# hohMiyazawa/hoh-ANS

Hardware: AMD Instinct MI355X
Metric: MB/s encode+decode (bit-exact) on 8-bit RGB, 1/2/4/8 MI355X; % HBM roofline (higher is better)
Workload: dtype u8; 1 GPU; 8192x8192 synthetic RGB (gradient + triangular noise k=4, seeds 1..32: one image each), 256x256 tiles, choh -s0 encode + dhoh decode, side index, 4 slot(s) x 8 image(s) per step (batched calls hoh_encode_images_async / hoh_decode_images_async) = 32 images in flight per GPU, 4 hardware queues; W=8192, H=8192, tiles=1024, per_gpu=8192x8192, batch=8, parallelism=1 GPU

## Files before the change

hoh-ans_amd/csrc/hoh_api.cpp:

```cpp
#include "hoh_internal.h"
#include "hoh_dec.h"
#include "hoh_index_blob.h"
#include "../../include/hoh_ans.h"

#include <math.h>
#include <string.h>
#include <stdlib.h>
#include <vector>
#include <algorithm>
#include <stdio.h>
#include <string>
#include <atomic>

void launch_synth(uint8_t* rgb, int W, int H, int y0, uint64_t seed, int noise, hipStream_t s);
void launch_natural(uint8_t* rgb, int W, int rows, int y0, uint64_t seed, hipStream_t s);
void launch_put_bytes(uint8_t* dst, const uint8_t* b, int n, hipStream_t s, int copies = 1, uint64_t stride = 0);
void launch_status_enc(const uint32_t* gerr, const uint64_t* total, uint64_t cap, uint64_t* out, hipStream_t s);
void launch_status_enc_batch(const uint32_t* gerr, const uint64_t* img_total, const uint32_t* img_err,
                             uint64_t stride, uint64_t* out, int n, hipStream_t s);

std::atomic<uint64_t> g_device_allocs{0};

namespace {

// ... 80 lines not shown
      c->sms[k] += v;
      c->scount[k] += 1;
    }
  }
  c->nmark = 0;
  c->knames.clear();
}

static void prof_mark(hoh_ctx* c, hipStream_t s, const char* name, bool reset) {
  if (!c->profiling) return;
  if (reset) prof_fold(c);
  if (c->nmark == c->kev.size()) {
    hipEvent_t e;
    if (hipEventCreate(&e) != hipSuccess) return;
    c->kev.push_back(e);
  }
  (void)hipEventRecord(c->kev[c->nmark++], s);
  c->knames.push_back(name);
}

struct Prof {
  hoh_ctx* c;
  hipStream_t s;
  Prof(hoh_ctx* c_, hipStream_t s_, bool async = false) : c(c_), s(s_) { prof_mark(c, s, "start", !async); }
  void mark(const char* name) { prof_mark(c, s, name, false); }
};

extern "C" {

const char* hoh_version(void) { return "hoh-ans_amd 0.2 (gfx950)"; }

uint64_t hoh_device_alloc_count(void) { return g_device_allocs.load(std::memory_order_relaxed); }

const char* hoh_strerror(int code) {
  switch (code) {
    case HOH_OK: return "ok";
    case HOH_E_ARG: return "invalid argument";
    case HOH_E_CAP: return "output capacity too small";
    case HOH_E_HIP: return "HIP runtime error";
    case HOH_E_RANGE: return "symbol / range / prob_bits outside the supported set";
    case HOH_E_UNREPRODUCIBLE: return "the reference emits uninitialised bytes for this input";
    case HOH_E_UNSUPPORTED: return "not implemented on this path";
    case HOH_E_CORRUPT: return "malformed or undecodable bitstream";
    case HOH_E_NODEV: return "no HIP device";
  }
  return "unknown error";
}

int hoh_ctx_create(hoh_ctx** out, int device) {
  if (!out) return HOH_E_ARG;
  *out = nullptr;
  int n = 0;
  if (hipGetDeviceCount(&n) != hipSuccess || n <= device || device < 0) return HOH_E_NODEV;
  if (hipSetDevice(device) != hipSuccess) return HOH_E_NODEV;
  {
    static std::atomic<int> warned{0};
    const char* q = getenv("GPU_MAX_HW_QUEUES");
    if (q && atoi(q) > 20 && !getenv("HOH_QUIET") && !warned.exchange(1))
      fprintf(stderr, "hoh: GPU_MAX_HW_QUEUES=%s: more than 20 hardware queues per process cost 15-30%% "
                      "throughput on MI355X; share queues between streams instead\n", q);
  }
  hoh_ctx* c = new hoh_ctx();
  c->device = device;
  if (hipDeviceGetAttribute(&c->cus, hipDeviceAttributeMultiprocessorCount, device) != hipSuccess || c->cus <= 0)
    c->cus = 256;
  if (hipStreamCreateWithFlags(&c->own, hipStreamNonBlocking) != hipSuccess) { delete c; return HOH_E_HIP; }
  if (hipHostMalloc((void**)&c->pinned, 4096) != hipSuccess) { delete c; return HOH_E_HIP; }
  *out = c;
  return HOH_OK;
}

static int lz_posting() { return HOH_KNOB(LZ_POSTING, 1); }

static void freebuf(Buf& b) { if (b.p) (void)hipFree(b.p); b.p = nullptr; b.n = 0; }

void hoh_ctx_destroy(hoh_ctx* c) {
  if (!c) return;
  (void)hipSetDevice(c->device);
  Buf* all[] = {&c->dbg, &c->idx8, &c->fpb, &c->lzs, &c->pinfo, &c->lg, &c->sym, &c->hist, &c->candbits, &c->matches, &c->lzspec, &c->pal, &c->streams, &c->tiles, &c->hdr,
                &c->tab_fast, &c->tab_gen, &c->slabs, &c->ckpt, &c->misc, &c->tsizes};
  for (Buf* b : all) freebuf(*b);
  for (Buf& b : c->scr.chunks) freebuf(b);
  dec_free(c->dec);
  for (auto e : c->kev) (void)hipEventDestroy(e);
  if (c->pinned) (void)hipHostFree(c->pinned);
  if (c->own) (void)hipStreamDestroy(c->own);
  if (c->side.s) (void)hipStreamDestroy(c->side.s);
  if (c->side.fork) (void)hipEventDestroy(c->side.fork);
  if (c->side.join) (void)hipEventDestroy(c->side.join);
  delete c;
}

void hoh_set_profiling(hoh_ctx* c, int on) { if (c) c->profiling = on; }

void* hoh_ctx_stream(hoh_ctx* c) { return c ? (void*)c->own : nullptr; }

int hoh_ctx_set_option(hoh_ctx* c, int option, int64_t value) {
  if (!c) return HOH_E_ARG;
  switch (option) {
    case HOH_OPT_NOIX_DECODER:
      if (value < HOH_NOIX_ADAPTIVE || value > HOH_NOIX_WAVE) return HOH_E_ARG;
      c->noix = (int)value;
      return HOH_OK;
    case HOH_OPT_DECODABLE:
      if (value != 0 && value != 1) return HOH_E_ARG;
      c->decodable = (int)value;
      return HOH_OK;
    case HOH_OPT_SMALL_IMAGES:
      if (value != 0 && value != 1) return HOH_E_ARG;
      c->small = (int)value;
      return HOH_OK;
    case HOH_OPT_CHAIN_TABLES:
      if (value < HOH_CHAIN_TABLES_AUTO || value > HOH_CHAIN_TABLES_GLOBAL) return HOH_E_ARG;
      c->chain_tables = (int)value;
      return HOH_OK;
  }
  return HOH_E_ARG;
}

int hoh_get_kernel_ms(hoh_ctx* c, const char** names, float* ms, int max) {
  if (!c || c->nmark < 2) return 0;
  int k = 0;
  (void)hipEventSynchronize(c->kev[c->nmark - 1]);
  for (size_t i = 1; i < c->nmark && k < max; i++, k++) {
    float v = 0;
    (void)hipEventElapsedTime(&v, c->kev[i - 1], c->kev[i]);
    if (names) names[k] = c->knames[i].c_str();
    if (ms) ms[k] = v;
  }
  return k;
}

int hoh_get_kernel_stats(hoh_ctx* c, const char** names, double* total_ms, uint64_t* count, int max) {
  if (!c) return 0;
  prof_fold(c);
  int k = 0;
  for (; k < (int)c->snames.size() && k < max; k++) {
    if (names) names[k] = c->snames[k].c_str();
    if (total_ms) total_ms[k] = c->sms[k];
    if (count) count[k] = c->scount[k];
  }
  return k;
}

#ifdef HOH_DEBUG_READ
extern "C" int hoh_debug_read(hoh_ctx* c, int which, void* dst, size_t bytes) {
  if (!c || !dst) return HOH_E_ARG;
  if (which == 2) {
    if (!c->dec.bufs[15] || bytes > c->dec.sizes[15]) return HOH_E_ARG;
    return hipMemcpy(dst, (const uint8_t*)c->dec.bufs[15] + c->dec.sizes[15] - bytes, bytes, hipMemcpyDeviceToHost) == hipSuccess
               ? HOH_OK : HOH_E_HIP;
  }
  const Buf& b = which == 0 ? c->matches : which == 3 ? c->lzs : which == 4 ? c->fpb : which == 5 ? c->dbg
               : which == 6 ? c->streams : c->lzspec;
  if (bytes > b.n || !b.p) return HOH_E_ARG;
  return hipMemcpy(dst, b.p, bytes, hipMemcpyDeviceToHost) == hipSuccess ? HOH_OK : HOH_E_HIP;
}
#endif

void hoh_reset_kernel_stats(hoh_ctx* c) {
  if (!c) return;
  prof_fold(c);
  c->snames.clear();
  c->sms.clear();
  c->scount.clear();
}

int hoh_tiling(int W, int H, int* xt, int* yt, int* tw, int* th) {
  if ((W >= 512 || H >= 512) && W >= 256 && H >= 256) {
    *xt = W / 256; *yt = H / 256;
    *tw = (W + *xt - 1) / *xt; *th = (H + *yt - 1) / *yt;
    return 1;
  }
  *xt = *yt = 1; *tw = W; *th = H;
  return 0;
}

size_t hoh_encode_bound(int W, int H) {
  int xt, yt, tw, th;
  hoh_tiling(W, H, &xt, &yt, &tw, &th);
  return 64 + (size_t)xt * yt * 3 + 5 * (size_t)W * H + (size_t)xt * yt * 4096;
}

static size_t header_fixed(int W, int H, uint8_t* o) {
  size_t p = 0;
  o[p++] = 153; o[p++] = 72; o[p++] = 79; o[p++] = 72;
  o[p++] = 2;
  o[p++] = 8;
  p = hoh_write_varint(o, (uint32_t)p, (uint64_t)W - 1);
  p = hoh_write_varint(o, (uint32_t)p, (uint64_t)H - 1);
  return p;
}

size_t hoh_file_prefix(int W, int H, const uint32_t* ts, int nt, uint8_t* out, size_t cap) {
  int xt, yt, tw, th;
  if (!hoh_tiling(W, H, &xt, &yt, &tw, &th) || nt != xt * yt) return 0;
  std::vector<uint8_t> b(32 + 3 * (size_t)nt);
  size_t p = header_fixed(W, H, b.data());
  b[p++] = (uint8_t)(xt - 1);
  b[p++] = (uint8_t)(yt - 1);
  for (int i = 0; i + 1 < nt; i++) p = hoh_write_varint(b.data(), (uint32_t)p, ts[i]);
  if (p > cap) return 0;
  memcpy(out, b.data(), p);
  return p;
}

int hoh_peek_header(const uint8_t* h, size_t size, int* W, int* H, int* xt, int* yt) {
  if (!h || size < 8 || h[0] != 153 || h[1] != 72 || h[2] != 79 || h[3] != 72) return HOH_E_CORRUPT;
  if (h[4] != 2 || h[5] != 8) return HOH_E_UNSUPPORTED;
  size_t p = 6;
  auto rv = [&](uint64_t& v) -> bool {
    if (p >= size) return false;
    uint64_t b0 = h[p++];
    if (!(b0 & 0x80)) { v = b0; return true; }
    if (p >= size) return false;
    uint64_t b1 = h[p++];
    if (!(b1 & 0x80)) { v = ((b0 & 0x7f) << 7) + b1; return true; }
    if (p >= size) return false;
    uint64_t b2 = h[p++];
    v = ((b0 & 0x7f) << 14) + ((b1 & 0x7f) << 7) + b2;
    return true;
  };
  uint64_t w, hh;
  if (!rv(w) || !rv(hh)) return HOH_E_CORRUPT;
  *W = (int)w + 1; *H = (int)hh + 1;
  int tw, th, x, y;
  hoh_tiling(*W, *H, &x, &y, &tw, &th);
  if (xt) *xt = x;
  if (yt) *yt = y;
  return HOH_OK;
}


static void prof_cb(void* p, const char* name) { ((Prof*)p)->mark(name); }

static int ensure_log2_tables(hoh_ctx* c, int W, int H, EncodeJob& j) {
  const int rw = W - (j.xt - 1) * j.tw, bh = H - (j.yt - 1) * j.th;
  uint32_t ns[4] = {(uint32_t)(j.tw * j.th), (uint32_t)(rw * j.th), (uint32_t)(j.tw * bh), (uint32_t)(rw * bh)};
  uint32_t un[4] = {0, 0, 0, 0};
  int nu = 0;
  for (int i = 0; i < 4; i++) {
    bool dup = false;
    for (int k = 0; k < nu; k++) dup |= un[k] == ns[i];
    if (!dup && ns[i]) un[nu++] = ns[i];
  }
  if (!(c->lg_key[0] == un[0] && c->lg_key[1] == un[1] && c->lg_key[2] == un[2] && c->lg_key[3] == un[3])) {
    std::vector<double> tab;
    for (int k = 0; k < nu; k++) {
      c->lg_off[k] = tab.size();
      for (uint32_t f = 0; f <= un[k] + 1; f++) tab.push_back(f ? -log2((double)f / (double)un[k]) : 0.0);
    }
    int e = ensure(c->lg, tab.size() * sizeof(double));
    if (e) return e;
    if (hipMemcpy(c->lg.p, tab.data(), tab.size() * sizeof(double), hipMemcpyHostToDevice) != hipSuccess) return HOH_E_HIP;
    for (int k = 0; k < 4; k++) c->lg_key[k] = un[k];
  }
  j.lg = (const double*)c->lg.p;
  for (int k = 0; k < 4; k++) { j.lg_n[k] = c->lg_key[k]; j.lg_off[k] = c->lg_off[k]; }
  return HOH_OK;
}

static int encode_tiles_impl(hoh_ctx* c, const uint8_t* d_rgb, int W, int H, int t0, int ntiles,
                             uint8_t* d_out, size_t cap, uint64_t prefix, int write_table,
                             uint32_t* d_tile_sizes, uint64_t* total_out, hoh_index* idx,
                             hipStream_t s, int speed = 0, uint64_t* d_status = nullptr, int nimg = 1,
                             uint64_t out_stride = 0, int small_n = 0) {
  const bool async = d_status != nullptr;
  int xt, yt, tw, th;
  hoh_tiling(W, H, &xt, &yt, &tw, &th);
  if (small_n > 0) { xt = 1; yt = small_n; tw = W; th = H / small_n; }
  if (tw > HOH_MAX_TILE_W || (size_t)tw * th > (1u << 24)) return HOH_E_UNSUPPORTED;
  if (speed && ((size_t)((tw + 39) / 40) * ((th + 39) / 40) > HOH_MAPCAP || tw > 1024)) return HOH_E_UNSUPPORTED;
  if (t0 < 0 || ntiles <= 0 || t0 + ntiles > xt * yt) return HOH_E_ARG;
  Prof prof(c, s, async);
  EncodeJob j{};
  memset(&j, 0, sizeof(j));
  j.speed = speed;
  j.decodable = c->decodable;
  j.chain_tables = c->chain_tables;
  j.spt = speed ? SPT_S : SK_PER_TILE;
  j.rgb = d_rgb; j.W = W; j.H = H;
  j.xt = xt; j.yt = yt; j.tw = tw; j.th = th;
  j.t0 = t0; j.ntiles = ntiles;
  j.npix_cap = (uint32_t)rup((size_t)tw * th, HOH_SEG > 64 ? 64 : 64);
  j.lz_cap = (uint32_t)rup(j.npix_cap / 4 + j.npix_cap / 255 + 16, 8);
  j.gen_stride = 512;
  j.hdr_cap = HOH_HDR_CAP;
  const size_t S = (size_t)ntiles * j.spt;
  if (!speed && S * HOH_FAST_STRIDE * sizeof(EncFast) > 0xffffffffull) return HOH_E_UNSUPPORTED;
  size_t nsym = (size_t)ntiles * 3 * (j.npix_cap + j.lz_cap) + (size_t)ntiles * j.npix_cap;
  size_t nslab = (size_t)ntiles * 3 * (j.npix_cap + 8 + j.lz_cap + 8) + (size_t)ntiles * (j.npix_cap + 8);
  if (speed) {
    nsym = sym_total_s(ntiles, j.npix_cap, j.lz_cap);
    nslab = slab_total_s(ntiles, j.npix_cap, j.lz_cap);
    j.tpool_off = nslab;
    j.tpool_words = HOH_KNOB(TRIAL_POOL, 1) ? (size_t)ntiles * HOH_NPLANE_S * (j.npix_cap / 2) : 0;
    nslab += j.tpool_words;
  }
  const size_t nck = speed ? 1 : S * (j.npix_cap / HOH_SEG + 2);
  int e = HOH_OK;
  if (speed) {
    if ((e = ensure(c->idx8, (size_t)ntiles * j.npix_cap))) return e;
    if ((e = ensure(c->fpb, (size_t)ntiles * j.npix_cap * 13))) return e;
    if ((e = ensure(c->pinfo, (size_t)ntiles * HOH_NPLANE_S * (sizeof(PlaneInfo) + 8 * 4)))) return e;
    if ((e = ensure_log2_tables(c, W, H, j))) return e;
    j.idx8 = (uint8_t*)c->idx8.p;
    j.fpb = (uint32_t*)c->fpb.p;
// ... 790 lines not shown
```

hoh-ans_amd/csrc/k_front.hip:

```cpp
#include "hoh_internal.h"

#define RING_SMALL 1040
#define RING_SMALL_MAX_W 271
#define RING 2048
#define RING_MAX_W 1200
#define WTAB 512
#define CSET 512
#define NT 256
#define PF 4

typedef unsigned short us2 __attribute__((ext_vector_type(2)));

__device__ __forceinline__ us2 as_us2(uint32_t v) { return __builtin_bit_cast(us2, v); }
__device__ __forceinline__ uint32_t as_u32(us2 v) { return __builtin_bit_cast(uint32_t, v); }

__device__ __forceinline__ uint16_t med16(uint16_t a, uint16_t b, uint16_t c) {
  if (a > b) return b > c ? b : (c > a ? a : c);
  return b < c ? b : (c > a ? c : a);
}

__device__ __forceinline__ uint32_t rb_form(uint32_t rgb) {
  const uint32_t g = (rgb >> 8) & 255u;
  return ((rgb & 0x00ff00ffu) | 0x01000100u) - g * 0x10001u;
}
// ... 216 lines not shown
    ti.mode = (fl & TF_GREY) ? 0 : 128;
    ti.pad = 0;
    j.tiles[t] = ti;
  }
}

__global__ __launch_bounds__(NT) void k_colours(EncodeJob j) {
  __shared__ uint32_t hset[CSET];
  __shared__ uint32_t hpos[CSET];
  __shared__ uint32_t pc[256], pp[256];
  __shared__ int s_ncol, s_np;
  const int t = blockIdx.x, tid = threadIdx.x;
  const int gt = j.t0 + t;
  const int x0 = (gt % j.xt) * j.tw, y0 = (gt / j.xt) * j.th;
  const int w = min(j.tw, j.W - x0), h = min(j.th, j.H - y0);
  const uint32_t npix = (uint32_t)w * h;
  const uint8_t* img = j.rgb + ((size_t)y0 * j.W + x0) * 3;
  const size_t pitch = (size_t)j.W * 3;
  for (int i = tid; i < CSET; i += NT) { hset[i] = 0xffffffffu; hpos[i] = 0xffffffffu; }
  if (tid == 0) { s_ncol = 0; s_np = 0; }
  uint32_t x = tid, y = 0;
  while (x >= (uint32_t)w) { x -= w; y++; }
  __syncthreads();
  const int lane = tid & 63;
  for (uint32_t q0 = 0; q0 < npix; q0 += 4 * NT) {
    uint32_t v[4];
#pragma unroll
    for (int u = 0; u < 4; u++) {
      const uint32_t q = q0 + (uint32_t)u * NT + tid;
      v[u] = 0xffffffffu;
      if (q < npix) {
        const uint8_t* p = img + (size_t)y * pitch + (size_t)x * 3;
        v[u] = p[0] | (p[1] << 8) | (p[2] << 16);
      }
      x += NT;
      while (x >= (uint32_t)w) { x -= w; y++; }
    }
#pragma unroll
    for (int u = 0; u < 4; u++) {
      const uint32_t q = q0 + (uint32_t)u * NT + tid;
      const uint32_t prev = (uint32_t)__builtin_amdgcn_update_dpp((int)v[u], (int)v[u], 0x138, 0xf, 0xf, false);
      if (q < npix && (lane == 0 || v[u] != prev) && *(volatile int*)&s_ncol <= 256) {
        uint32_t hsh = (v[u] * 2654435761u) >> 23;
        for (int probe = 0; probe < CSET; probe++) {
          const uint32_t old = atomicCAS(&hset[hsh], 0xffffffffu, v[u]);
          if (old == 0xffffffffu) { atomicAdd(&s_ncol, 1); atomicMin(&hpos[hsh], q); break; }
          if (old == v[u]) { atomicMin(&hpos[hsh], q); break; }
          hsh = (hsh + 1) & (CSET - 1);
        }
      }
    }
    __syncthreads();
    if (s_ncol > 256) break;
  }
  if (s_ncol > 256) {
    if (tid == 0) j.ncol[t] = -1;
    return;
  }
  for (int i = tid; i < CSET; i += NT) {
    if (hset[i] != 0xffffffffu) {
      const int k = atomicAdd(&s_np, 1);
      pc[k] = hset[i];
      pp[k] = hpos[i];
    }
  }
  __syncthreads();
  if (tid < s_np) {
    const uint32_t me = pp[tid];
    uint32_t rank = 0;
    for (int m = 0; m < s_np; m++) rank += pp[m] < me;
    j.palette[(size_t)t * 256 + rank] = pc[tid];
  }
  if (tid == 0) j.ncol[t] = s_ncol;
}

template <uint32_t RG>
__global__ __launch_bounds__(NT) void k_front(EncodeJob j) {
  __shared__ uint32_t ring[2 * RG + 4];
  front_tile<true, RG>(j, ring);
}

__global__ __launch_bounds__(NT) void k_front_wide(EncodeJob j) { front_tile<false, 1>(j, nullptr); }

__device__ __forceinline__ void palette_tile(const EncodeJob& j, int t, uint32_t* hk, uint32_t* hv, uint32_t* phist);

__global__ __launch_bounds__(NT) void k_palette(EncodeJob j) {
  __shared__ uint32_t hk[1024];
  __shared__ uint32_t hv[1024];
  __shared__ uint32_t phist[256];
  for (int t = blockIdx.x; t < j.ntiles; t += gridDim.x) {
    palette_tile(j, t, hk, hv, phist);
    __syncthreads();
  }
}

__device__ __forceinline__ void palette_tile(const EncodeJob& j, int t, uint32_t* hk, uint32_t* hv, uint32_t* phist) {
  const int tid = threadIdx.x;
  const TileInfo ti = j.tiles[t];
  if (!(ti.flags & TF_PALETTE_CAND) || (ti.flags & TF_GREY)) return;
  const int w = ti.w, h = ti.h, ncol = ti.colours;
  const uint32_t npix = (uint32_t)w * h;
  for (int i = tid; i < 1024; i += NT) hk[i] = 0xffffffffu;
  phist[tid] = 0;
  __syncthreads();
  if (tid < ncol) {
    const uint32_t c = j.palette[(size_t)t * 256 + tid];
    uint32_t hsh = (c * 2654435761u) >> 22;
    while (atomicCAS(&hk[hsh], 0xffffffffu, c) != 0xffffffffu) hsh = (hsh + 1) & 1023;
    hv[hsh] = (uint32_t)tid;
  }
  __syncthreads();
  uint16_t* pl = j.sym + med_plane_off(j, t, 3);
  const uint8_t* img = j.rgb + ((size_t)ti.y0 * j.W + ti.x0) * 3;
  const size_t pitch = (size_t)j.W * 3;
  int x = tid, y = 0;
  while (x >= w) { x -= w; y++; }
  for (uint32_t q = tid; q < npix; q += NT) {
    const uint8_t* p = img + (size_t)y * pitch + (size_t)x * 3;
    const uint32_t c = p[0] | (p[1] << 8) | (p[2] << 16);
    uint32_t hsh = (c * 2654435761u) >> 22;
    for (int probe = 0; probe < 1024 && hk[hsh] != c; probe++) hsh = (hsh + 1) & 1023;
    pl[q] = (uint16_t)hv[hsh];
    if (j.idx8) j.idx8[(size_t)t * j.npix_cap + q] = (uint8_t)hv[hsh];
    x += NT;
    while (x >= w) { x -= w; y++; }
  }
  __syncthreads();
  const uint32_t nblk = (npix + NT - 1) / NT;
  for (int b = (int)nblk - 1; b >= 0; b--) {
    const uint32_t q = (uint32_t)b * NT + tid;
    uint32_t r = 0;
    if (q < npix) {
      const uint32_t qx = q % (uint32_t)w, qy = q / (uint32_t)w;
      const uint16_t v = pl[q];
      const uint16_t L = qx ? pl[q - 1] : (uint16_t)128;
      const uint16_t T = qy ? pl[q - w] : (uint16_t)128;
      const uint16_t TL = (qx && qy) ? pl[q - w - 1] : (uint16_t)128;
      r = ((int)v - (int)med16(T, L, (uint16_t)(T + L - TL)) + 128 + 256) & 255;
    }
    __syncthreads();
    if (q < npix) { pl[q] = (uint16_t)r; atomicAdd(&phist[r], 1u); }
    __syncthreads();
  }
  uint32_t* hs = j.hist + (size_t)(t * j.spt + med_kind(j, 3)) * 512;
  for (int i = tid; i < 512; i += NT) hs[i] = i < 256 ? phist[i] : 0u;
}

void launch_palette(const EncodeJob& j, hipStream_t s) {
  hipLaunchKernelGGL(k_palette, dim3(j.ntiles < 128 ? j.ntiles : 128), dim3(NT), 0, s, j);
}

#define F2_TAB 256
#define F2_RING 256

__device__ __forceinline__ uint32_t wshl1(uint32_t v, uint32_t old) {
  return (uint32_t)__builtin_amdgcn_update_dpp((int)old, (int)v, 0x130, 0xf, 0xf, false);
}
__device__ __forceinline__ uint32_t wshr1(uint32_t v, uint32_t old) {
  return (uint32_t)__builtin_amdgcn_update_dpp((int)old, (int)v, 0x138, 0xf, 0xf, false);
}
__device__ __forceinline__ uint32_t lane_of(uint32_t v, int l) { return __builtin_amdgcn_readlane(v, l); }

__device__ __forceinline__ uint32_t wt_find(const uint32_t* key, uint32_t k) {
  uint32_t sl = (k >> 1) & (F2_TAB - 1);
  for (int probe = 0; probe < F2_TAB; probe++) {
    const uint32_t o = key[sl];
    if (o == k) return sl;
    if (o == 0u) return F2_TAB;
    sl = (sl + 1) & (F2_TAB - 1);
  }
  return F2_TAB;
}

__device__ __forceinline__ uint32_t wt_put(uint32_t* key, uint32_t k) {
  uint32_t sl = (k >> 1) & (F2_TAB - 1);
  for (int probe = 0; probe < F2_TAB; probe++) {
    const uint32_t old = atomicCAS(&key[sl], 0u, k);
    if (old == 0u || old == k) return sl;
    sl = (sl + 1) & (F2_TAB - 1);
  }
  return F2_TAB;
}

__device__ __forceinline__ void wt_max(uint32_t* pos, uint32_t sl, uint32_t v) {
  __hip_atomic_fetch_max(&pos[sl], v, __ATOMIC_RELAXED, __HIP_MEMORY_SCOPE_WORKGROUP);
}

__global__ __launch_bounds__(NT) void k_front256(EncodeJob j) {
  __shared__ uint32_t tab[4][2][F2_TAB + 1];
  __shared__ uint32_t tpos[4][2][F2_TAB + 1];
  __shared__ uint32_t pring[4][F2_RING];
#ifndef F2_HC
#define F2_HC 1
#endif
#ifndef F2_AGG
#define F2_AGG 0
#endif
  __shared__ uint32_t hist[F2_HC][3 * 512 - 256 + 64 * F2_AGG];
  __shared__ int s_notgrey, s_ncand;
  const int t = blockIdx.x, tid = threadIdx.x, lane = tid & 63, wv = tid >> 6;
  const int gt = j.t0 + t;
  const int x0 = (gt % j.xt) * 256, y0 = (gt / j.xt) * 256;
  const uint32_t npix = 256u * 256u;
  for (int i = tid; i < F2_HC * (3 * 512 - 256 + 64 * F2_AGG); i += NT) (&hist[0][0])[i] = 0;
  uint32_t* hl = hist[lane & (F2_HC - 1)];
  for (int i = lane; i < 2 * (F2_TAB + 1); i += 64) tab[wv][i / (F2_TAB + 1)][i % (F2_TAB + 1)] = 0;
  for (int i = lane; i < 2 * (F2_TAB + 1); i += 64) tpos[wv][i / (F2_TAB + 1)][i % (F2_TAB + 1)] = 0;
  if (tid == 0) { s_notgrey = 0; s_ncand = 0; }
  uint16_t* res0 = j.sym + med_plane_off(j, t, 0);
  uint16_t* res1 = j.sym + med_plane_off(j, t, 1);
  uint16_t* res2 = j.sym + med_plane_off(j, t, 2);
  uint64_t* cand = j.candbits + (size_t)t * (j.npix_cap / 64);
  const uint8_t* img = j.rgb + ((size_t)y0 * j.W + x0) * 3;
  const size_t pitch = (size_t)j.W * 3;
  const bool lz = j.speed == 0 && !(j.exp & 2);
  uint32_t* ring = pring[wv];
  auto load_row = [&](int y, uint32_t* o) {
#pragma unroll
    for (int k = 0; k < 4; k++) {
      const int x = 64 * k + lane;
      const uint8_t* p = img + (size_t)y * pitch + (size_t)x * 3;
      uint32_t v;
      __builtin_memcpy(&v, x ? p - 1 : p, 4);
      o[k] = x ? (v >> 8) : (v & 0xffffffu);
    }
  };
  const uint32_t GREY = 0x808080u;
  const int ya = 64 * wv, yb = ya + 64;
  uint32_t prow[4], cur[4], nxt[4];
  if (ya > 0) load_row(ya - 1, prow);
  else { prow[0] = prow[1] = prow[2] = prow[3] = GREY; }
  load_row(ya, cur);
  load_row(ya + 1, nxt);
  __syncthreads();
  uint32_t notgrey = 0;
  int ncand = 0;
  int cb = 0;
  uint32_t slot_prev = F2_TAB;
  if (lz) {
    if (ya > 0) {
      const uint32_t pv = prow[3];
      const uint32_t a1 = wshl1(pv, lane_of(cur[0], 0));
      const uint32_t a2 = wshl1(a1, lane_of(cur[0], 1));
      const uint32_t a3 = wshl1(a2, lane_of(cur[0], 2));
      const uint32_t k = fp32(pv, a1, a2, a3);
      slot_prev = wt_put(tab[wv][1], k);
      if (slot_prev < F2_TAB) wt_max(tpos[wv][1], slot_prev, lane);
      ring[(uint32_t)(ya * 256 - 64 + lane) & (F2_RING - 1)] = pv;
    }
    ring[(uint32_t)(ya * 256 + lane) & (F2_RING - 1)] = cur[0];
  }
  for (int y = ya; y < yb; y++) {
    const bool hasT = y > 0;
#pragma unroll
    for (int k = 0; k < 4; k++) {
      const uint32_t q = (uint32_t)y * 256u + 64u * k + lane;
      const uint32_t v = cur[k];
      const uint32_t g = (v >> 8) & 255u;
      notgrey |= (v ^ (g * 0x010101u)) & 0xffffffu;
      const uint32_t lft = k ? lane_of(cur[k - 1], 63) : GREY;
      const uint32_t tlf = k ? lane_of(prow[k - 1], 63) : GREY;
      const uint32_t vL = wshr1(v, lft);
      const uint32_t vT = hasT ? prow[k] : GREY;
      const uint32_t vTL = hasT ? wshr1(prow[k], tlf) : GREY;
      const uint32_t gL = (vL >> 8) & 255u, gT = (vT >> 8) & 255u, gTL = (vTL >> 8) & 255u;
      const uint32_t gg = (gT + gL - gTL) & 0xffffu;
      const uint32_t pg = max(min(gT, gL), min(max(gT, gL), gg));
      const uint32_t rg = (g - pg + 128u) & 255u;
      const us2 tt = as_us2(rb_form(vT)), ll = as_us2(rb_form(vL)), tl = as_us2(rb_form(vTL));
      const us2 gr = tt + ll - tl;
      const us2 mn = __builtin_elementwise_min(tt, ll), mx = __builtin_elementwise_max(tt, ll);
      const us2 pr = __builtin_elementwise_max(mn, __builtin_elementwise_min(mx, gr));
      const uint32_t rrb = as_u32(as_us2(rb_form(v)) - pr + (us2)(256)) & 0x01ff01ffu;
      const uint32_t rr = rrb & 0xffffu, rb = rrb >> 16;
      res0[q] = (uint16_t)rg;
      res1[q] = (uint16_t)rr;
      res2[q] = (uint16_t)rb;
#if F2_AGG
      auto hadd = [&](uint32_t i) {
        const uint32_t i0 = __builtin_amdgcn_readfirstlane(i);
        const uint32_t n0 = (uint32_t)__popcll(__ballot(i == i0));
        const bool dup = i == i0 && lane != 0;
        atomicAdd(&hl[dup ? 3 * 512 - 256 + lane : i], lane == 0 ? n0 : dup ? 0u : 1u);
      };
      hadd(rg);
      hadd(256 + rr);
      hadd(768 + rb);
#else
      atomicAdd(&hl[rg], 1u);
      atomicAdd(&hl[256 + rr], 1u);
      atomicAdd(&hl[768 + rb], 1u);
#endif
      if (!lz) continue;
      const uint32_t nx = k < 3 ? cur[k + 1] : nxt[0];
      const uint32_t v1 = wshl1(v, lane_of(nx, 0));
      const uint32_t v2 = wshl1(v1, lane_of(nx, 1));
      const uint32_t v3 = wshl1(v2, lane_of(nx, 2));
      ring[(q + 64u) & (F2_RING - 1)] = (q + 64u < npix) ? nx : 0u;
      const bool win = q + 3 < npix;
      const uint32_t hq = win ? fp32(v, v1, v2, v3) : 0u;
      uint32_t* tc = tab[wv][cb];
      uint32_t* pc = tpos[wv][cb];
      const uint32_t* tp = tab[wv][cb ^ 1];
      const uint32_t* pp = tpos[wv][cb ^ 1];
#if F2_AGG
      const uint32_t h0 = __builtin_amdgcn_readfirstlane(hq);
      const uint64_t m0 = __ballot(hq == h0);
      const bool kdup = hq == h0 && lane != 0;
      uint32_t sq = hq && !kdup ? wt_put(tc, hq) : F2_TAB;
      {
        const uint32_t s0 = __builtin_amdgcn_readfirstlane(sq);
        if (kdup) sq = s0;
      }
      if (sq < F2_TAB && !kdup) wt_max(pc, sq, 63u - lane);
#else
      const uint32_t sq = hq ? wt_put(tc, hq) : F2_TAB;
      const bool kdup = false;
      const uint64_t m0 = 1;
      if (sq < F2_TAB) wt_max(pc, sq, 63u - lane);
#endif
      const uint32_t sp = hq ? wt_find(tp, hq) : F2_TAB;
      const uint32_t fcur = sq < F2_TAB ? 63u - pc[sq] : 64u;
      const uint32_t lprev = sp < F2_TAB ? pp[sp] : 0u;
      const bool ccur = fcur < (uint32_t)lane, cprev = sp < F2_TAB && lprev >= (uint32_t)lane;
      const uint64_t flag = __ballot(ccur || cprev);
      uint64_t word = 0;
      if (flag) {
        auto same = [&](uint32_t p) {
          return ring[p & (F2_RING - 1)] == v && ring[(p + 1) & (F2_RING - 1)] == v1 &&
                 ring[(p + 2) & (F2_RING - 1)] == v2 && ring[(p + 3) & (F2_RING - 1)] == v3;
        };
        const uint32_t q0 = q - lane;
        bool c = false, full = false;
        if (ccur || cprev) {
          c = same(ccur ? q0 + fcur : q0 - 64u + lprev);
          if (!c && ccur && cprev) c = same(q0 - 64u + lprev);
          full = !c;
        }
        if (__ballot(full)) {
          if (full) {
            const uint32_t bmax = q < 64 ? q : 64;
            for (uint32_t b = 1; b <= bmax && !c; b++) c = same(q - b);
          }
        }
        word = __ballot(c);
      }
      if (sq < F2_TAB && !kdup) { pc[sq] = 0; wt_max(pc, sq, lane ? (uint32_t)lane : 63u - (uint32_t)__builtin_clzll(m0)); }
      if (lane == 0) cand[q >> 6] = word;
      ncand += lane == 0 ? __popcll(word) : 0;
      uint32_t* tpw = tab[wv][cb ^ 1];
      tpw[slot_prev] = 0;
      tpos[wv][cb ^ 1][slot_prev] = 0;
      slot_prev = kdup ? F2_TAB : sq;
      cb ^= 1;
    }
#pragma unroll
    for (int k = 0; k < 4; k++) { prow[k] = cur[k]; cur[k] = nxt[k]; }
    if (y + 2 < 256) load_row(y + 2, nxt);
  }
  if (notgrey) atomicOr(&s_notgrey, 1);
  if (ncand) atomicAdd(&s_ncand, ncand);
  __syncthreads();
  for (int i = tid; i < 3 * 512; i += NT) {
    const int k = i / 512, sv = i % 512;
    uint32_t v = 0;
#pragma unroll
    for (int hc = 0; hc < F2_HC; hc++) v += k == 0 ? (sv < 256 ? hist[hc][sv] : 0u) : hist[hc][k * 512 - 256 + sv];
    j.hist[(size_t)(t * j.spt + med_kind(j, k)) * 512 + sv] = v;
  }
  if (tid == 0) {
    TileInfo ti;
    ti.x0 = x0; ti.y0 = y0; ti.w = 256; ti.h = 256;
    ti.colours = j.ncol[t];
    uint32_t fl = 0;
    if (!s_notgrey) fl |= TF_GREY;
    if (!s_notgrey && ti.colours != -1 && ti.colours <= 2) fl |= TF_BINARY;
    if (!s_notgrey && !(fl & TF_BINARY)) fl |= TF_UNREPRODUCIBLE;
    if (s_notgrey && ti.colours != -1) fl |= TF_PALETTE_CAND;
    if (j.decodable) fl = 0;
    ti.flags = fl;
    ti.nmatch = 0;
    ti.ncand = (uint32_t)s_ncand;
    ti.size = 0; ti.lz_bytes = 0; ti.off = 0;
    ti.mode = (fl & TF_GREY) ? 0 : 128;
    ti.pad = 0;
    j.tiles[t] = ti;
  }
}

void launch_front(const EncodeJob& j, hipStream_t s) {
  hipLaunchKernelGGL(k_colours, dim3(j.ntiles), dim3(NT), 0, s, j);
  if (j.tw == 256 && j.th == 256) hipLaunchKernelGGL(k_front256, dim3(j.ntiles), dim3(NT), 0, s, j);
  else if (j.tw <= RING_SMALL_MAX_W) hipLaunchKernelGGL(k_front<RING_SMALL>, dim3(j.ntiles), dim3(NT), 0, s, j);
  else if (j.tw <= RING_MAX_W) hipLaunchKernelGGL(k_front<RING>, dim3(j.ntiles), dim3(NT), 0, s, j);
  else hipLaunchKernelGGL(k_front_wide, dim3(j.ntiles), dim3(NT), 0, s, j);
}
```

Baseline: 175,200 MB/s.

## Add bloom-filter fast path for LZ candidate detection in k_front256

Replaces the per-step open-addressing hash table probe with a cheap per-wave bit filter (two bits per 4-pixel fingerprint) in shared memory. When only a few lanes hit the filter, candidates are resolved exactly using ballot comparisons; when many hit, the wave falls back to the original hash-table path and returns to the filter after a run of quiet steps. This aims to cut atomicCAS/probe traffic on noisy tiles where repeats are rare. The cost is added control divergence and mode-switch bookkeeping, and candidate bits must stay exact to keep output bit-identical.

```diff
diff --git a/hoh-ans_amd/csrc/hoh_api.cpp b/hoh-ans_amd/csrc/hoh_api.cpp
--- a/hoh-ans_amd/csrc/hoh_api.cpp
+++ b/hoh-ans_amd/csrc/hoh_api.cpp
@@ -256,7 +256,7 @@
                ? HOH_OK : HOH_E_HIP;
   }
   const Buf& b = which == 0 ? c->matches : which == 3 ? c->lzs : which == 4 ? c->fpb : which == 5 ? c->dbg
-               : which == 6 ? c->streams : c->lzspec;
+               : which == 6 ? c->streams : which == 7 ? c->candbits : which == 8 ? c->tiles : c->lzspec;
   if (bytes > b.n || !b.p) return HOH_E_ARG;
   return hipMemcpy(dst, b.p, bytes, hipMemcpyDeviceToHost) == hipSuccess ? HOH_OK : HOH_E_HIP;
 }
diff --git a/hoh-ans_amd/csrc/k_front.hip b/hoh-ans_amd/csrc/k_front.hip
--- a/hoh-ans_amd/csrc/k_front.hip
+++ b/hoh-ans_amd/csrc/k_front.hip
@@ -392,6 +392,16 @@
 
 #define F2_TAB 256
 #define F2_RING 256
+#define F2_SCR (2 * (F2_TAB + 1))
+#ifndef F2_MLOG2
+#define F2_MLOG2 14
+#endif
+#ifndef F2_THR
+#define F2_THR 4
+#endif
+#ifndef F2_QUIET
+#define F2_QUIET 8
+#endif
 
 __device__ __forceinline__ uint32_t wshl1(uint32_t v, uint32_t old) {
   return (uint32_t)__builtin_amdgcn_update_dpp((int)old, (int)v, 0x130, 0xf, 0xf, false);
@@ -426,10 +436,21 @@
   __hip_atomic_fetch_max(&pos[sl], v, __ATOMIC_RELAXED, __HIP_MEMORY_SCOPE_WORKGROUP);
 }
 
-__global__ __launch_bounds__(NT) void k_front256(EncodeJob j) {
-  __shared__ uint32_t tab[4][2][F2_TAB + 1];
-  __shared__ uint32_t tpos[4][2][F2_TAB + 1];
+__device__ __forceinline__ uint32_t pmix(uint32_t v) {
+  const uint32_t m = (uint32_t)__umul24(v, 0x9E3779u);
+  return m ^ (m >> 15);
+}
+
+__global__ __launch_bounds__(NT) void k_front256(EncodeJob j, uint32_t kn) {
+  __shared__ uint32_t scr[4][2 * F2_SCR];
   __shared__ uint32_t pring[4][F2_RING];
+#ifdef HOH_KNOBS
+  const uint32_t mlog2 = kn & 31u, thr = (kn >> 5) & 127u, quietk = kn >> 13;
+  bool tmode = (kn >> 12) & 1u;
+#else
+  constexpr uint32_t mlog2 = F2_MLOG2, thr = F2_THR, quietk = F2_QUIET;
+  bool tmode = false;
+#endif
 #ifndef F2_HC
 #define F2_HC 1
 #endif
@@ -444,8 +465,11 @@
   const uint32_t npix = 256u * 256u;
   for (int i = tid; i < F2_HC * (3 * 512 - 256 + 64 * F2_AGG); i += NT) (&hist[0][0])[i] = 0;
   uint32_t* hl = hist[lane & (F2_HC - 1)];
-  for (int i = lane; i < 2 * (F2_TAB + 1); i += 64) tab[wv][i / (F2_TAB + 1)][i % (F2_TAB + 1)] = 0;
-  for (int i = lane; i < 2 * (F2_TAB + 1); i += 64) tpos[wv][i / (F2_TAB + 1)][i % (F2_TAB + 1)] = 0;
+  uint32_t* const sw = scr[wv];
+  for (int i = lane; i < 2 * F2_SCR; i += 64) sw[i] = 0;
+  auto tabp = [&](int c) { return sw + c * (F2_TAB + 1); };
+  auto posp = [&](int c) { return sw + F2_SCR + c * (F2_TAB + 1); };
+  auto fltp = [&](int c) { return sw + ((uint32_t)c << (mlog2 - 5)); };
   if (tid == 0) { s_notgrey = 0; s_ncand = 0; }
   uint16_t* res0 = j.sym + med_plane_off(j, t, 0);
   uint16_t* res1 = j.sym + med_plane_off(j, t, 1);
@@ -477,18 +501,46 @@
   int ncand = 0;
   int cb = 0;
   uint32_t slot_prev = F2_TAB;
+  auto fbit = [&](uint32_t m0, uint32_t mn) -> uint32_t {
+    const uint32_t m1 = wshl1(m0, lane_of(mn, 0));
+    const uint32_t m2 = wshl1(m1, lane_of(mn, 1));
+    const uint32_t m3 = wshl1(m2, lane_of(mn, 2));
+    const uint32_t f = m0 + __builtin_rotateleft32(m1, 9) + __builtin_rotateleft32(m2, 18) + __builtin_rotateleft32(m3, 27);
+    return (uint32_t)__umul24(f ^ (f >> 13), 0xC2B2AFu);
+  };
+  auto fword = [&](uint32_t h) { return h >> (37 - mlog2); };
+  auto fmask = [&](uint32_t h) { return 1u << ((h >> (32 - mlog2)) & 31) | 1u << ((h >> (27 - mlog2)) & 31); };
+  auto table_start = [&](uint32_t q, uint32_t xp, uint32_t v, bool has_prev) {
+    cb = 0;
+    slot_prev = F2_TAB;
+    if (has_prev) {
+      const uint32_t a1 = wshl1(xp, lane_of(v, 0));
+      const uint32_t a2 = wshl1(a1, lane_of(v, 1));
+      const uint32_t a3 = wshl1(a2, lane_of(v, 2));
+      slot_prev = wt_put(tabp(1), fp32(xp, a1, a2, a3));
+      if (slot_prev < F2_TAB) wt_max(posp(1), slot_prev, lane);
+      ring[(q - 64u) & (F2_RING - 1)] = xp;
+    }
+    ring[q & (F2_RING - 1)] = v;
+  };
+  int fb = 0;
+  uint32_t wprev = 0;
+  uint32_t quiet = 0;
+  uint32_t mcur = pmix(cur[0]);
+#ifdef HOH_DEBUG_READ
+  uint32_t n_clean = 0, n_res = 0, n_tab = 0, n_to_tab = 0, n_to_fast = 0;
+#define F2_COUNT(x) ((x)++)
+#else
+#define F2_COUNT(x) ((void)0)
+#endif
   if (lz) {
-    if (ya > 0) {
-      const uint32_t pv = prow[3];
-      const uint32_t a1 = wshl1(pv, lane_of(cur[0], 0));
-      const uint32_t a2 = wshl1(a1, lane_of(cur[0], 1));
-      const uint32_t a3 = wshl1(a2, lane_of(cur[0], 2));
-      const uint32_t k = fp32(pv, a1, a2, a3);
-      slot_prev = wt_put(tab[wv][1], k);
-      if (slot_prev < F2_TAB) wt_max(tpos[wv][1], slot_prev, lane);
-      ring[(uint32_t)(ya * 256 - 64 + lane) & (F2_RING - 1)] = pv;
-    }
-    ring[(uint32_t)(ya * 256 + lane) & (F2_RING - 1)] = cur[0];
+    if (tmode) {
+      table_start((uint32_t)(ya * 256 + lane), prow[3], cur[0], ya > 0);
+    } else if (ya > 0) {
+      const uint32_t fh = fbit(pmix(prow[3]), mcur);
+      wprev = fword(fh);
+      atomicOr(&fltp(1)[wprev], fmask(fh));
+    }
   }
   for (int y = ya; y < yb; y++) {
     const bool hasT = y > 0;
@@ -533,71 +585,142 @@
 #endif
       if (!lz) continue;
       const uint32_t nx = k < 3 ? cur[k + 1] : nxt[0];
-      const uint32_t v1 = wshl1(v, lane_of(nx, 0));
-      const uint32_t v2 = wshl1(v1, lane_of(nx, 1));
-      const uint32_t v3 = wshl1(v2, lane_of(nx, 2));
-      ring[(q + 64u) & (F2_RING - 1)] = (q + 64u < npix) ? nx : 0u;
+      const uint32_t mnx = pmix(nx);
+      const uint32_t q0 = (uint32_t)y * 256u + 64u * k;
       const bool win = q + 3 < npix;
-      const uint32_t hq = win ? fp32(v, v1, v2, v3) : 0u;
-      uint32_t* tc = tab[wv][cb];
-      uint32_t* pc = tpos[wv][cb];
-      const uint32_t* tp = tab[wv][cb ^ 1];
-      const uint32_t* pp = tpos[wv][cb ^ 1];
+      uint64_t word = 0;
+      if (!tmode) {
+        const uint32_t xp = k ? cur[k - 1] : prow[3];
+        uint32_t* fc = fltp(fb);
+        uint32_t* fp = fltp(fb ^ 1);
+        const uint32_t fh = fbit(mcur, mnx);
+        const uint32_t wi = fword(fh), bits = win ? fmask(fh) : 0u;
+        const uint32_t seen = atomicOr(&fc[wi], bits) | fp[wi];
+        const uint64_t bal = __ballot(win && (seen & bits) == bits);
+        if (bal) {
+          if ((uint32_t)__popcll(bal) <= thr) {
+            F2_COUNT(n_res);
+            const uint64_t winm = __ballot(win);
+            uint64_t cm = 0, todo = bal;
+            while (todo) {
+              const int lf = __builtin_ctzll(todo);
+              todo &= todo - 1;
+              if ((cm >> lf) & 1) continue;
+              uint64_t mx = q0 ? ~0ull : 0ull, my = ~0ull;
+#pragma unroll
+              for (int i = 0; i < 4; i++) {
+                const int l = lf + i;
+                const uint32_t p = l < 64 ? (uint32_t)__builtin_amdgcn_readlane(v, l)
+                                          : (uint32_t)__builtin_amdgcn_readlane(nx, l - 64);
+                const uint64_t X = __ballot(xp == p), Y = __ballot(v == p), Z = __ballot(nx == p);
+                mx &= i ? (X >> i) | (Y << (64 - i)) : X;
+                my &= i ? (Y >> i) | (Z << (64 - i)) : Y;
+              }
+              if ((mx >> lf) | (my & ((1ull << lf) - 1))) cm |= 1ull << lf;
+              cm |= my & (~1ull << lf) & winm;
+            }
+            word = cm;
+          } else {
+            fc[wi] = 0;
+            fp[wprev] = 0;
+            table_start(q, xp, v, q0 != 0);
+            tmode = true;
+            quiet = 0;
+            F2_COUNT(n_to_tab);
+          }
+        } else {
+          F2_COUNT(n_clean);
+        }
+        if (!tmode) {
+          fp[wprev] = 0;
+          wprev = wi;
+          fb ^= 1;
+        }
+      }
+      if (tmode) {
+        F2_COUNT(n_tab);
+        const uint32_t v1 = wshl1(v, lane_of(nx, 0));
+        const uint32_t v2 = wshl1(v1, lane_of(nx, 1));
+        const uint32_t v3 = wshl1(v2, lane_of(nx, 2));
+        ring[(q + 64u) & (F2_RING - 1)] = (q + 64u < npix) ? nx : 0u;
+        const uint32_t hq = win ? fp32(v, v1, v2, v3) : 0u;
+        uint32_t* tc = tabp(cb);
+        uint32_t* pc = posp(cb);
+        const uint32_t* tp = tabp(cb ^ 1);
+        const uint32_t* pp = posp(cb ^ 1);
 #if F2_AGG
-      const uint32_t h0 = __builtin_amdgcn_readfirstlane(hq);
-      const uint64_t m0 = __ballot(hq == h0);
-      const bool kdup = hq == h0 && lane != 0;
-      uint32_t sq = hq && !kdup ? wt_put(tc, hq) : F2_TAB;
-      {
-        const uint32_t s0 = __builtin_amdgcn_readfirstlane(sq);
-        if (kdup) sq = s0;
+        const uint32_t h0 = __builtin_amdgcn_readfirstlane(hq);
+        const uint64_t m0 = __ballot(hq == h0);
+        const bool kdup = hq == h0 && lane != 0;
+        uint32_t sq = hq && !kdup ? wt_put(tc, hq) : F2_TAB;
+        {
+          const uint32_t s0 = __builtin_amdgcn_readfirstlane(sq);
+          if (kdup) sq = s0;
+        }
+        if (sq < F2_TAB && !kdup) wt_max(pc, sq, 63u - lane);
+#else
+        const uint32_t sq = hq ? wt_put(tc, hq) : F2_TAB;
+        const bool kdup = false;
+        const uint64_t m0 = 1;
+        if (sq < F2_TAB) wt_max(pc, sq, 63u - lane);
+#endif
+        const uint32_t sp = hq ? wt_find(tp, hq) : F2_TAB;
+        const uint32_t fcur = sq < F2_TAB ? 63u - pc[sq] : 64u;
+        const uint32_t lprev = sp < F2_TAB ? pp[sp] : 0u;
+        const bool ccur = fcur < (uint32_t)lane, cprev = sp < F2_TAB && lprev >= (uint32_t)lane;
+        const uint64_t flag = __ballot(ccur || cprev);
+        if (flag) {
+          auto same = [&](uint32_t p) {
+            return ring[p & (F2_RING - 1)] == v && ring[(p + 1) & (F2_RING - 1)] == v1 &&
+                   ring[(p + 2) & (F2_RING - 1)] == v2 && ring[(p + 3) & (F2_RING - 1)] == v3;
+          };
+          bool c = false, full = false;
+          if (ccur || cprev) {
+            c = same(ccur ? q0 + fcur : q0 - 64u + lprev);
+            if (!c && ccur && cprev) c = same(q0 - 64u + lprev);
+            full = !c;
+          }
+          if (__ballot(full)) {
+            if (full) {
+              const uint32_t bmax = q < 64 ? q : 64;
+              for (uint32_t b = 1; b <= bmax && !c; b++) c = same(q - b);
+            }
+          }
+          word = __ballot(c);
+        }
+        if (sq < F2_TAB && !kdup) { pc[sq] = 0; wt_max(pc, sq, lane ? (uint32_t)lane : 63u - (uint32_t)__builtin_clzll(m0)); }
+        tabp(cb ^ 1)[slot_prev] = 0;
+        posp(cb ^ 1)[slot_prev] = 0;
+        slot_prev = kdup ? F2_TAB : sq;
+        cb ^= 1;
+        quiet = word ? 0u : quiet + 1u;
+        if (quiet >= quietk) {
+          tabp(cb ^ 1)[slot_prev] = 0;
+          posp(cb ^ 1)[slot_prev] = 0;
+          const uint32_t fh = fbit(mcur, mnx);
+          wprev = fword(fh);
+          fb = 0;
+          atomicOr(&fltp(1)[wprev], win ? fmask(fh) : 0u);
+          tmode = false;
+          F2_COUNT(n_to_fast);
+        }
       }
-      if (sq < F2_TAB && !kdup) wt_max(pc, sq, 63u - lane);
-#else
-      const uint32_t sq = hq ? wt_put(tc, hq) : F2_TAB;
-      const bool kdup = false;
-      const uint64_t m0 = 1;
-      if (sq < F2_TAB) wt_max(pc, sq, 63u - lane);
-#endif
-      const uint32_t sp = hq ? wt_find(tp, hq) : F2_TAB;
-      const uint32_t fcur = sq < F2_TAB ? 63u - pc[sq] : 64u;
-      const uint32_t lprev = sp < F2_TAB ? pp[sp] : 0u;
-      const bool ccur = fcur < (uint32_t)lane, cprev = sp < F2_TAB && lprev >= (uint32_t)lane;
-      const uint64_t flag = __ballot(ccur || cprev);
-      uint64_t word = 0;
-      if (flag) {
-        auto same = [&](uint32_t p) {
-          return ring[p & (F2_RING - 1)] == v && ring[(p + 1) & (F2_RING - 1)] == v1 &&
-                 ring[(p + 2) & (F2_RING - 1)] == v2 && ring[(p + 3) & (F2_RING - 1)] == v3;
-        };
-        const uint32_t q0 = q - lane;
-        bool c = false, full = false;
-        if (ccur || cprev) {
-          c = same(ccur ? q0 + fcur : q0 - 64u + lprev);
-          if (!c && ccur && cprev) c = same(q0 - 64u + lprev);
-          full = !c;
-        }
-        if (__ballot(full)) {
-          if (full) {
-            const uint32_t bmax = q < 64 ? q : 64;
-            for (uint32_t b = 1; b <= bmax && !c; b++) c = same(q - b);
-          }
-        }
-        word = __ballot(c);
-      }
-      if (sq < F2_TAB && !kdup) { pc[sq] = 0; wt_max(pc, sq, lane ? (uint32_t)lane : 63u - (uint32_t)__builtin_clzll(m0)); }
       if (lane == 0) cand[q >> 6] = word;
       ncand += lane == 0 ? __popcll(word) : 0;
-      uint32_t* tpw = tab[wv][cb ^ 1];
-      tpw[slot_prev] = 0;
-      tpos[wv][cb ^ 1][slot_prev] = 0;
-      slot_prev = kdup ? F2_TAB : sq;
-      cb ^= 1;
+      mcur = mnx;
     }
 #pragma unroll
     for (int k = 0; k < 4; k++) { prow[k] = cur[k]; cur[k] = nxt[k]; }
     if (y + 2 < 256) load_row(y + 2, nxt);
   }
+#ifdef HOH_DEBUG_READ
+  if (j.dbg && lane == 0) {
+    uint32_t* d = j.dbg + (size_t)t * 64 + 56;
+    atomicAdd(&d[0], n_clean); atomicAdd(&d[1], n_res); atomicAdd(&d[2], n_tab);
+    atomicAdd(&d[3], n_to_tab); atomicAdd(&d[4], n_to_fast);
+  }
+#endif
+#undef F2_COUNT
   if (notgrey) atomicOr(&s_notgrey, 1);
   if (ncand) atomicAdd(&s_ncand, ncand);
   __syncthreads();
@@ -630,7 +753,15 @@
 
 void launch_front(const EncodeJob& j, hipStream_t s) {
   hipLaunchKernelGGL(k_colours, dim3(j.ntiles), dim3(NT), 0, s, j);
-  if (j.tw == 256 && j.th == 256) hipLaunchKernelGGL(k_front256, dim3(j.ntiles), dim3(NT), 0, s, j);
+  if (j.tw == 256 && j.th == 256) {
+    const int mode = HOH_KNOB(F2_MODE, 0);
+    auto clamp = [](int v, int lo, int hi) { return (uint32_t)(v < lo ? lo : v > hi ? hi : v); };
+    const uint32_t mlog2 = clamp(HOH_KNOB(F2_MLOG2, F2_MLOG2), 6, 14);
+    const uint32_t thr = mode == 1 ? 64u : clamp(HOH_KNOB(F2_THR, F2_THR), 0, 64);
+    const uint32_t quiet = mode == 2 ? 0x7ffffu : clamp(HOH_KNOB(F2_QUIET, F2_QUIET), 1, 0x7ffff);
+    const uint32_t kn = mlog2 | thr << 5 | (mode == 2 ? 1u << 12 : 0u) | quiet << 13;
+    hipLaunchKernelGGL(k_front256, dim3(j.ntiles), dim3(NT), 0, s, j, kn);
+  }
   else if (j.tw <= RING_SMALL_MAX_W) hipLaunchKernelGGL(k_front<RING_SMALL>, dim3(j.ntiles), dim3(NT), 0, s, j);
   else if (j.tw <= RING_MAX_W) hipLaunchKernelGGL(k_front<RING>, dim3(j.ntiles), dim3(NT), 0, s, j);
   else hipLaunchKernelGGL(k_front_wide, dim3(j.ntiles), dim3(NT), 0, s, j);
```

New measurement: 200,000 MB/s, median of 6. +14.2%, better.
